# unslothai/unsloth

Measured on AMD Instinct MI355X. Metric: train tokens/sec, Llama-3-8B QLoRA (NF4) r=16 seq2048 bf16, higher is better.
Workload: dtype bf16; 1 GPU; Llama-3-8B QLoRA NF4 r=16 (q,k,v,o,gate,up,down) seq2048 bf16, fwd+bwd+AdamW; model=Llama-3-8B (synthetic weights), global_batch=4, seq_len=2048, parallelism=dp1, layers=32, lora_rank=16, gradient_checkpointing=unsloth, gc_schedule_chosen=all (every layer keeps everything), nf4_decoded_weight_mirrors=off (every NF4 weight is decoded at every use INSIDE the timed step), trainable_params=41943040, attention=csrc/attention.hip (causal GQA flash, fwd+bwd), optimizer=FlatAdamW fp32 on LoRA params

## Files before the change

### unsloth_amd/csrc/lora_side.hip

```cpp
#include "common.h"

typedef __attribute__((ext_vector_type(2))) __bf16 bf16x2_t;
typedef __attribute__((ext_vector_type(2))) _Float16 f16x2_t;

#define UAMD_TN_MAX_PROBLEMS 8

namespace {

constexpr int TN_COLS = 128;
constexpr int TN_R = 16;

struct TnArgs {
    int n_probs;
    int M;
    int S;
    int rows_per_wave;
    int total_slabs;
    int slab_start[UAMD_TN_MAX_PROBLEMS + 1];
    int64_t ws_off[UAMD_TN_MAX_PROBLEMS];
    float* ws;
    uamd_lora_tn_problem p[UAMD_TN_MAX_PROBLEMS];
};

typedef __attribute__((ext_vector_type(8))) __bf16 bf16x8_t;
typedef __attribute__((ext_vector_type(8))) _Float16 f16x8_t;
typedef __attribute__((ext_vector_type(4))) float f32x4_t;
typedef __attribute__((ext_vector_type(4))) short s16x4_t;
typedef __attribute__((address_space(3))) s16x4_t lds_s16x4;
typedef __attribute__((address_space(3))) unsigned char lds_u8;

template <typename T> struct Mfma16;
template <> struct Mfma16<bf16_t> {
    typedef bf16x8_t frag;
    static __device__ __forceinline__ f32x4_t run(frag a, frag b, f32x4_t c) {
        return __builtin_amdgcn_mfma_f32_16x16x32_bf16(a, b, c, 0, 0, 0);
    }
};
template <> struct Mfma16<f16_t> {
    typedef f16x8_t frag;
    static __device__ __forceinline__ f32x4_t run(frag a, frag b, f32x4_t c) {
        return __builtin_amdgcn_mfma_f32_16x16x32_f16(a, b, c, 0, 0, 0);
    }
};

constexpr int TN_ZT = 32 * 256;
constexpr int TN_PT = 32 * 64;
constexpr int TN_STAGE = TN_ZT + TN_PT;
#ifndef UAMD_TN_STAGES
#define UAMD_TN_STAGES 2
#endif
#ifndef UAMD_TN_RPW_MAX
#define UAMD_TN_RPW_MAX 512
#endif
#ifndef UAMD_TN_MIN_WAVES
#define UAMD_TN_MIN_WAVES 4096
#endif
constexpr int TN_NST = UAMD_TN_STAGES;
static_assert(TN_NST >= 2 && TN_NST <= 4, "ring of 2..4 stages (4 x 4 x 10 KiB = the 160 KiB of a CU)");
constexpr int TN_WAVE_LDS = TN_NST * TN_STAGE;

__device__ __forceinline__ void tn_dma(const void* gptr, unsigned lds_dst) {
    unsigned keep;
    asm volatile(
        "s_mov_b32 %0, m0\n\t"
        "s_mov_b32 m0, %2\n\t"
        "s_nop 0\n\t"
        "global_load_lds_dwordx4 %1, off\n\t"
        "s_mov_b32 m0, %0"
        : "=&s"(keep)
        : "v"(gptr), "s"(lds_dst)
        : "memory");
}

template <typename T>
__global__ void __launch_bounds__(256) lora_tn_kernel(TnArgs a) {
    extern __shared__ __attribute__((aligned(16))) unsigned char smem[];
    typedef typename Mfma16<T>::frag frag_t;
    const int tid = threadIdx.x, lane = tid & 63;
    const int wave = __builtin_amdgcn_readfirstlane(tid >> 6);
    const int64_t unit = (int64_t)blockIdx.x * 4 + wave;
    if (unit >= (int64_t)a.total_slabs * a.S) return;
    const int slab_lin = (int)(unit % a.total_slabs);
    const int sblk = (int)(unit / a.total_slabs);
    int pi = 0;
#pragma unroll
    for (int i = 1; i < UAMD_TN_MAX_PROBLEMS; ++i)
        if (i < a.n_probs && slab_lin >= a.slab_start[i]) pi = i;
    const uamd_lora_tn_problem& pr = a.p[pi];
    const int slab = slab_lin - a.slab_start[pi];
    const int n_slabs = a.slab_start[pi + 1] - a.slab_start[pi];
    const int M = a.M, N = pr.N, R = pr.R;
    const T* Z = (const T*)pr.Z;
    const float* P = pr.P;
    unsigned char* my = smem + wave * TN_WAVE_LDS;
    const unsigned my_lds = (unsigned)(uintptr_t)(lds_u8*)my;

    const int zr4 = lane >> 4;
    int zcol[8];
#pragma unroll
    for (int i = 0; i < 8; ++i) {
        const int row = 4 * i + zr4;
        const int f = (row & 3) | (((row >> 3) & 1) << 2);
        const int u16 = ((((lane & 15) >> 1) ^ f) << 1) | (lane & 1);
        int col = slab * TN_COLS + u16 * 8;
        if (col + 8 > N) col = N - 8;
        zcol[i] = col;
    }
    const int prow = lane >> 2;
    const int pc = (lane & 3) * 4 + 4 <= ((R + 3) & ~3) ? (lane & 3) * 4 : 0;
    auto issue = [&](int m0, int stage) {
        const unsigned d = my_lds + stage * TN_STAGE;
#pragma unroll
        for (int i = 0; i < 8; ++i) {
            int row = m0 + 4 * i + zr4;
            row = row < M ? row : M - 1;
            tn_dma(Z + (int64_t)row * pr.ldz + zcol[i], d + i * 1024);
        }
#pragma unroll
        for (int i = 0; i < 2; ++i) {
            int row = m0 + 16 * i + prow;
            row = row < M ? row : M - 1;
            tn_dma(P + (int64_t)row * pr.ldp + pc, d + TN_ZT + i * 1024);
        }
    };

    const int l15 = lane & 15, g4 = lane >> 4;
    const int sg2 = l15 >> 2;
    const int f_rd = sg2 | ((g4 & 1) << 2);
    const int z_lane = (8 * g4 + sg2) * 256 + f_rd * 32 + (l15 & 3) * 8;
    const int p_lane = TN_ZT + (8 * g4) * 64 + l15 * 4;

    f32x4_t acc[8];
#pragma unroll
    for (int j = 0; j < 8; ++j) acc[j] = f32x4_t{0.f, 0.f, 0.f, 0.f};

    const int m_base = sblk * a.rows_per_wave;
    const int m_end = min(m_base + a.rows_per_wave, M);
    const int nch = (m_end - m_base + 31) / 32;
#pragma unroll
    for (int i = 0; i < TN_NST - 1; ++i)
        if (i < nch) issue(m_base + 32 * i, i);
    for (int ch = 0; ch < nch; ++ch) {
        const int m0 = m_base + ch * 32;
        const int stage = ch % TN_NST;
        if (ch + TN_NST - 1 < nch) {
            issue(m0 + 32 * (TN_NST - 1), (ch + TN_NST - 1) % TN_NST);
            if (TN_NST == 2) asm volatile("s_waitcnt vmcnt(10)" ::: "memory");
            else if (TN_NST == 3) asm volatile("s_waitcnt vmcnt(20)" ::: "memory");
            else asm volatile("s_waitcnt vmcnt(30)" ::: "memory");
        } else {
            const int younger = nch - 1 - ch;
            if (younger >= 2) asm volatile("s_waitcnt vmcnt(20)" ::: "memory");
            else if (younger == 1) asm volatile("s_waitcnt vmcnt(10)" ::: "memory");
            else asm volatile("s_waitcnt vmcnt(0)" ::: "memory");
        }
        const unsigned char* sz = my + stage * TN_STAGE;
        union { T e[8]; frag_t f; } pa;
#pragma unroll
        for (int e = 0; e < 8; ++e) {
            float x = *reinterpret_cast<const float*>(sz + p_lane + e * 64);
            if (m0 + 8 * g4 + e >= M || l15 >= R) x = 0.f;
            pa.e[e] = from_f32<T>(x);
        }
#pragma unroll
        for (int jt = 0; jt < 8; ++jt) {
            union { s16x4_t h[2]; frag_t f; } zb;
            const int a0 = z_lane ^ (jt * 32);
            zb.h[0] = __builtin_amdgcn_ds_read_tr16_b64_v4i16((lds_s16x4*)(sz + a0));
            zb.h[1] = __builtin_amdgcn_ds_read_tr16_b64_v4i16((lds_s16x4*)(sz + a0 + 4 * 256));
            acc[jt] = Mfma16<T>::run(pa.f, zb.f, acc[jt]);
        }
    }

    const int64_t npad = (int64_t)n_slabs * TN_COLS;
    float* part = a.ws + a.ws_off[pi] + (int64_t)sblk * TN_R * npad + slab * TN_COLS + l15;
#pragma unroll
    for (int jt = 0; jt < 8; ++jt)
#pragma unroll
        for (int r = 0; r < 4; ++r) part[(int64_t)(4 * g4 + r) * npad + jt * 16] = acc[jt][r];
}

__global__ void __launch_bounds__(256) lora_tn_reduce_kernel(TnArgs a) {
    const int pi = blockIdx.y;
    const uamd_lora_tn_problem& pr = a.p[pi];
    const int n_slabs = a.slab_start[pi + 1] - a.slab_start[pi];
    const int64_t npad = (int64_t)n_slabs * TN_COLS;
    const int64_t idx = (int64_t)blockIdx.x * 256 + threadIdx.x;
    const int N = pr.N, R = pr.R;
    if (idx >= (int64_t)R * N) return;
    const int r = (int)(idx / N), n = (int)(idx - (int64_t)r * N);
    const float* part = a.ws + a.ws_off[pi] + (int64_t)r * npad + n;
    float v = 0.f;
    const int64_t sstride = (int64_t)TN_R * npad;
    int s = 0;
    for (; s + 8 <= a.S; s += 8) {
        float t[8];
#pragma unroll
        for (int u = 0; u < 8; ++u) t[u] = part[(int64_t)(s + u) * sstride];
#pragma unroll
        for (int u = 0; u < 8; ++u) v += t[u];
    }
    for (; s < a.S; ++s) v += part[(int64_t)s * sstride];
    v *= pr.scale;
    float* o = (pr.out_nr & 1) ? pr.out + (int64_t)n * pr.ldo + r : pr.out + (int64_t)r * pr.ldo + n;
    *o = (pr.out_nr & 2) ? *o + v : v;
}

constexpr int XA_KS = 64;
constexpr int XA_XT = 32 * XA_KS * 2;
template <int NT> struct XaCfg {
    static constexpr int WT = NT * 16 * XA_KS * 2;
    static constexpr int STAGE = XA_XT + WT;
    static constexpr int WAVE = 2 * STAGE;
    static constexpr int RED = 4 * 32 * NT * 16 * 4;
    static constexpr int LDS = 4 * WAVE > RED ? 4 * WAVE : RED;
};

template <typename T, int NT>
__global__ void __launch_bounds__(256) lora_xa2_kernel(const T* __restrict__ X, int64_t ldx,
                                                       const T* __restrict__ W, int64_t ldw,
                                                       float* __restrict__ out, int64_t ld_out,
                                                       T* __restrict__ out_k, int64_t ld_k, int k_cols,
                                                       int M, int K, int R, int out_cols) {
    extern __shared__ __attribute__((aligned(16))) unsigned char smem[];
    typedef typename Mfma16<T>::frag frag_t;
    typedef XaCfg<NT> C;
    const int tid = threadIdx.x, lane = tid & 63;
    const int wave = __builtin_amdgcn_readfirstlane(tid >> 6);
    const int l15 = lane & 15, g4 = lane >> 4;
    const int m0 = blockIdx.x * 32;
    unsigned char* my = smem + wave * C::WAVE;
    const unsigned my_lds = (unsigned)(uintptr_t)(lds_u8*)my;

    const int nsteps_all = (K + XA_KS - 1) / XA_KS;
    const int s_beg = (nsteps_all * wave) / 4, s_end = (nsteps_all * (wave + 1)) / 4;

    const int drow = lane >> 3;
    int xoff[4], woff[2 * NT];
    int xslot[4];
#pragma unroll
    for (int i = 0; i < 4; ++i) {
        const int row = 8 * i + drow;
        xslot[i] = (lane & 7) ^ ((row >> 1) & 7);
        int gm = m0 + row;
        gm = gm < M ? gm : M - 1;
        xoff[i] = gm;
    }
    int wslot[2 * NT];
#pragma unroll
    for (int i = 0; i < 2 * NT; ++i) {
        const int row = 8 * i + drow;
        wslot[i] = (lane & 7) ^ ((row >> 1) & 7);
        woff[i] = row < R ? row : R - 1;
    }
    auto issue = [&](int step, int stage) {
        const unsigned d = my_lds + stage * C::STAGE;
        const int k0 = step * XA_KS;
#pragma unroll
        for (int i = 0; i < 4; ++i) {
            int k = k0 + xslot[i] * 8;
            k = k + 8 <= K ? k : K - 8;
            tn_dma(X + (int64_t)xoff[i] * ldx + k, d + i * 1024);
        }
#pragma unroll
        for (int i = 0; i < 2 * NT; ++i) {
            int k = k0 + wslot[i] * 8;
            k = k + 8 <= K ? k : K - 8;
            tn_dma(W + (int64_t)woff[i] * ldw + k, d + XA_XT + i * 1024);
        }
    };

    f32x4_t acc[2][NT];
#pragma unroll
    for (int i = 0; i < 2; ++i)
#pragma unroll
        for (int j = 0; j < NT; ++j) acc[i][j] = f32x4_t{0.f, 0.f, 0.f, 0.f};

    const int sw = (l15 >> 1) & 7;
    const int f_lane = l15 * 128;
    constexpr int NDMA = 4 + 2 * NT;
    const int nst = s_end - s_beg;
    const int rot = nst > 0 ? (int)(blockIdx.x % nst) : 0;
    auto step_of = [&](int i) { const int j = i + rot; return s_beg + (j >= nst ? j - nst : j); };
    if (nst > 0) issue(step_of(0), 0);
    for (int it = 0; it < nst; ++it) {
        const int st = step_of(it);
        const int stage = it & 1;
        if (it + 1 < nst) {
            issue(step_of(it + 1), stage ^ 1);
            if (NDMA == 6) asm volatile("s_waitcnt vmcnt(6)" ::: "memory");
            else if (NDMA == 8) asm volatile("s_waitcnt vmcnt(8)" ::: "memory");
            else if (NDMA == 10) asm volatile("s_waitcnt vmcnt(10)" ::: "memory");
            else asm volatile("s_waitcnt vmcnt(12)" ::: "memory");
        } else {
            asm volatile("s_waitcnt vmcnt(0)" ::: "memory");
        }
        const unsigned char* sx = my + stage * C::STAGE;
        const unsigned char* swt = sx + XA_XT;
        const bool tail = st * XA_KS + XA_KS > K;
#pragma unroll
        for (int ks = 0; ks < 2; ++ks) {
            const int slot = ((4 * ks + g4) ^ sw) * 16;
            union FU { uint4 r; frag_t f; };
            FU xa[2], wb[NT];
#pragma unroll
            for (int i = 0; i < 2; ++i) xa[i].r = *reinterpret_cast<const uint4*>(sx + i * 2048 + f_lane + slot);
#pragma unroll
            for (int j = 0; j < NT; ++j) wb[j].r = *reinterpret_cast<const uint4*>(swt + j * 2048 + f_lane + slot);
            if (tail) {
                if (st * XA_KS + ks * 32 + g4 * 8 + 8 > K) {
#pragma unroll
                    for (int i = 0; i < 2; ++i) xa[i].r = make_uint4(0, 0, 0, 0);
                }
            }
#pragma unroll
            for (int i = 0; i < 2; ++i)
#pragma unroll
                for (int j = 0; j < NT; ++j) acc[i][j] = Mfma16<T>::run(xa[i].f, wb[j].f, acc[i][j]);
        }
    }

    __syncthreads();
    float* red = reinterpret_cast<float*>(smem);
#pragma unroll
    for (int i = 0; i < 2; ++i)
#pragma unroll
        for (int j = 0; j < NT; ++j)
#pragma unroll
            for (int r = 0; r < 4; ++r)
                red[(wave * 32 + i * 16 + 4 * g4 + r) * (NT * 16) + j * 16 + l15] = acc[i][j][r];
    __syncthreads();
    if (out != nullptr) {
        for (int idx = tid; idx < 32 * out_cols; idx += 256) {
            const int mm = idx / out_cols, c = idx - mm * out_cols;
            if (m0 + mm < M) {
                float v = 0.f;
                if (c < R) {
                    const float* q = red + mm * (NT * 16) + c;
                    v = ((q[0] + q[32 * NT * 16]) + q[2 * 32 * NT * 16]) + q[3 * 32 * NT * 16];
                }
                out[(int64_t)(m0 + mm) * ld_out + c] = v;
            }
        }
    }
    if (out_k != nullptr) {
        const int vec_per_row = k_cols >> 3;
        for (int idx = tid; idx < 32 * vec_per_row; idx += 256) {
            const int mm = idx / vec_per_row, c0 = (idx - mm * vec_per_row) * 8;
            if (m0 + mm < M) {
                Vec16<T> v;
#pragma unroll
                for (int j = 0; j < 8; ++j) {
                    const int c = c0 + j;
                    float x = 0.f;
                    if (c < R) {
                        const float* q = red + mm * (NT * 16) + c;
                        x = ((q[0] + q[32 * NT * 16]) + q[2 * 32 * NT * 16]) + q[3 * 32 * NT * 16];
                    }
                    v.e[j] = from_f32<T>(x);
                }
                st16(out_k + (int64_t)(m0 + mm) * ld_k + c0, v);
            }
        }
    }
}

template <typename T, int NT>
int launch_xa2(const void* X, int64_t ldx, const void* W, int64_t ldw, float* out, int64_t ld_out, void* out_k,
               int64_t ld_k, int k_cols, int M, int K, int R, int out_cols, hipStream_t st) {
    return uamd_launch_lds<&lora_xa2_kernel<T, NT>>(dim3((unsigned)((M + 31) / 32)), dim3(256), XaCfg<NT>::LDS, st, (const T*)X, ldx,
                                                    (const T*)W, ldw, out, ld_out, (T*)out_k, ld_k, k_cols, M, K, R, out_cols);
}

template <typename T>
int xa2_dispatch(const void* X, int64_t ldx, const void* W, int64_t ldw, float* out, int64_t ld_out, void* out_k,
                 int64_t ld_k, int k_cols, int M, int K, int R, int out_cols, hipStream_t st) {
    const int nt = (R + 15) / 16;
    if (nt <= 1) return launch_xa2<T, 1>(X, ldx, W, ldw, out, ld_out, out_k, ld_k, k_cols, M, K, R, out_cols, st);
    if (nt <= 2) return launch_xa2<T, 2>(X, ldx, W, ldw, out, ld_out, out_k, ld_k, k_cols, M, K, R, out_cols, st);
    if (nt <= 3) return launch_xa2<T, 3>(X, ldx, W, ldw, out, ld_out, out_k, ld_k, k_cols, M, K, R, out_cols, st);
    if (nt <= 4) return launch_xa2<T, 4>(X, ldx, W, ldw, out, ld_out, out_k, ld_k, k_cols, M, K, R, out_cols, st);
    return UAMD_ERR_ARG;
}

}

extern "C" int uamd_lora_tn(const uamd_lora_tn_problem* probs, int n_probs, int M, float* workspace,
                            int64_t workspace_floats, int dtype, void* stream) {
    if (!probs || n_probs < 1 || n_probs > UAMD_TN_MAX_PROBLEMS || M < 0 || !workspace) return UAMD_ERR_ARG;
    if (M == 0) return UAMD_OK;
    TnArgs a;
    a.n_probs = n_probs; a.M = M; a.ws = workspace;
    {
        int64_t slabs_all = 0;
        for (int i = 0; i < n_probs; ++i) slabs_all += (probs[i].N + TN_COLS - 1) / TN_COLS;
        int rpw = UAMD_TN_RPW_MAX;
        while (rpw > 128 && slabs_all * ((M + rpw - 1) / rpw) < UAMD_TN_MIN_WAVES) rpw >>= 1;
        a.rows_per_wave = rpw;
        a.S = (M + rpw - 1) / rpw;
    }
    int slabs = 0;
    int64_t off = 0;
    int max_rn_blocks = 1;
    for (int i = 0; i < UAMD_TN_MAX_PROBLEMS; ++i) {
        a.slab_start[i] = slabs;
        if (i < n_probs) {
            const uamd_lora_tn_problem& p = probs[i];
            if (!p.P || !p.Z || !p.out || p.N <= 0 || p.R <= 0 || p.R > TN_R) return UAMD_ERR_ARG;
            if ((p.N & 7) || p.N < 8 || (p.ldz & 7) || (p.ldp & 3) || !aligned16(p.Z) || !aligned16(p.P)) return UAMD_ERR_ALIGN;
            a.p[i] = p;
            a.ws_off[i] = off;
            const int ns = (p.N + TN_COLS - 1) / TN_COLS;
            slabs += ns;
            off += (int64_t)a.S * TN_R * ns * TN_COLS;
            const int64_t rn = ((int64_t)p.R * p.N + 255) / 256;
            if (rn > max_rn_blocks) max_rn_blocks = (int)rn;
        } else {
            a.p[i] = probs[0];
            a.ws_off[i] = 0;
        }
    }
    a.slab_start[UAMD_TN_MAX_PROBLEMS] = slabs;
    for (int i = n_probs; i < UAMD_TN_MAX_PROBLEMS; ++i) a.slab_start[i + 1] = slabs;
    a.total_slabs = slabs;
    if (off > workspace_floats) return UAMD_ERR_ARG;
    const int64_t blocks = ((int64_t)slabs * a.S + 3) / 4;
    if (blocks > 0x7fffffffLL) return UAMD_ERR_ARG;
    hipStream_t st = (hipStream_t)stream;
    UAMD_DISPATCH_HALF(dtype,
        if (int rc = uamd_launch_lds<&lora_tn_kernel<T>>(dim3((unsigned)blocks), dim3(256), 4 * TN_WAVE_LDS, st, a)) return rc)
    hipLaunchKernelGGL(lora_tn_reduce_kernel, dim3((unsigned)max_rn_blocks, (unsigned)n_probs), dim3(256), 0, st, a);
    return uamd_launch_status();
}

extern "C" int uamd_lora_xa2k(const void* X, int64_t ldx, const void* W, int64_t ldw, float* out, int64_t ld_out,
                              void* out_k, int64_t ld_k, int k_cols, int M, int K, int R, int out_cols, int dtype,
                              void* stream) {
    if (M < 0 || K < 8 || R <= 0 || R > 64) return UAMD_ERR_ARG;
    if (!out && !out_k) return UAMD_ERR_ARG;
    if (out && (out_cols < R || out_cols > 256)) return UAMD_ERR_ARG;
    if (out_k && (k_cols < R || k_cols > 256)) return UAMD_ERR_ARG;
    if (M == 0) return UAMD_OK;
    if ((K & 7) || (ldx & 7) || (ldw & 7) || !aligned16(X) || !aligned16(W)) return UAMD_ERR_ALIGN;
    if (out_k && ((k_cols & 7) || (ld_k & 7) || !aligned16(out_k))) return UAMD_ERR_ALIGN;
    UAMD_DISPATCH_HALF(dtype, return xa2_dispatch<T>(X, ldx, W, ldw, out, ld_out, out_k, ld_k, k_cols, M, K, R, out_cols, (hipStream_t)stream))
    return UAMD_ERR_DTYPE;
}

extern "C" int uamd_lora_xa2(const void* X, int64_t ldx, const void* W, int64_t ldw, float* out, int64_t ld_out,
                             int M, int K, int R, int out_cols, int dtype, void* stream) {
    if (!out) return UAMD_ERR_ARG;
    return uamd_lora_xa2k(X, ldx, W, ldw, out, ld_out, nullptr, 0, 0, M, K, R, out_cols, dtype, stream);
}

namespace {
template <typename T>
__global__ void __launch_bounds__(256) lora_prepare_kernel(const uamd_lora_prep_desc* __restrict__ d, int n_mats,
                                                          const int* __restrict__ tile_prefix) {
    __shared__ float tile[32][33];
    int lo = 0, hi = n_mats - 1;
    const int bid = blockIdx.x;
    while (lo < hi) {
        const int mid = (lo + hi + 1) >> 1;
        if (tile_prefix[mid] <= bid) lo = mid; else hi = mid - 1;
    }
    const uamd_lora_prep_desc m = d[lo];
    const int t = bid - tile_prefix[lo];
    const int tiles_c = (m.cols + 31) / 32;
    const int r0 = (t / tiles_c) * 32, c0 = (t % tiles_c) * 32;
    const int tx = threadIdx.x & 31, ty = threadIdx.x >> 5;
    const float* src = (const float*)m.src;
    T* rm = (T*)m.dst_rowmajor;
    T* tr = (T*)m.dst_transposed;
    T* pad = (T*)m.dst_pad;
    const bool pad_t = m.pad_transposed != 0;
#pragma unroll
    for (int i = 0; i < 4; ++i) {
        const int r = r0 + ty + 8 * i, c = c0 + tx;
        float v = 0.f;
        if (r < m.rows && c < m.cols) {
            v = src[(int64_t)r * m.cols + c];
            if (rm) rm[(int64_t)r * m.cols + c] = from_f32<T>(v);
            if (pad && !pad_t) pad[(int64_t)r * m.pad_ld + c] = from_f32<T>(m.pad_scale * v);
        }
        tile[ty + 8 * i][tx] = v;
    }
    __syncthreads();
    if (tr || (pad && pad_t)) {
#pragma unroll
        for (int i = 0; i < 4; ++i) {
            const int c = c0 + ty + 8 * i, r = r0 + tx;
            if (r < m.rows && c < m.cols) {
                const float v = tile[tx][ty + 8 * i];
                if (tr) tr[(int64_t)c * m.rows + r] = from_f32<T>(v);
                if (pad && pad_t) pad[(int64_t)c * m.pad_ld + r] = from_f32<T>(m.pad_scale * v);
            }
        }
    }
}
}

extern "C" int uamd_lora_prepare(const uamd_lora_prep_desc* descs_dev, const int* tile_prefix_dev, int n_mats,
                                 int total_tiles, int dtype, void* stream) {
    if (!descs_dev || !tile_prefix_dev || n_mats <= 0 || total_tiles < 0) return UAMD_ERR_ARG;
    if (total_tiles == 0) return UAMD_OK;
    hipStream_t st = (hipStream_t)stream;
    UAMD_DISPATCH_HALF(dtype, hipLaunchKernelGGL((lora_prepare_kernel<T>), dim3((unsigned)total_tiles), dim3(256), 0, st, descs_dev, n_mats,
                                                 tile_prefix_dev))
    return uamd_launch_status();
}
```

Baseline: 37580 tokens/s.

## Group LoRA TN problems sharing the same Z operand into one walk

When three LoRA weight-gradient problems share the same Z matrix (e.g. q/k/v using the same input activations), the TN kernel now streams Z through LDS once and runs three MFMA accumulators against it. The extra P operands are loaded straight from global memory into registers. This cuts redundant Z reads and the number of waves, at the cost of more registers (3x8 accumulators plus P values) and fewer units to spread across the GPU. A tuning bit can switch the grouping off.

```diff
diff --git a/unsloth_amd/csrc/lora_side.hip b/unsloth_amd/csrc/lora_side.hip
--- a/unsloth_amd/csrc/lora_side.hip
+++ b/unsloth_amd/csrc/lora_side.hip
@@ -10,13 +10,17 @@
 constexpr int TN_COLS = 128;
 constexpr int TN_R = 16;
 
+constexpr int TN_GROUP = 3;
+
 struct TnArgs {
     int n_probs;
+    int n_walks;
     int M;
     int S;
     int rows_per_wave;
     int total_slabs;
-    int slab_start[UAMD_TN_MAX_PROBLEMS + 1];
+    int walk_start[UAMD_TN_MAX_PROBLEMS + 1];
+    int walk_mem[UAMD_TN_MAX_PROBLEMS];
     int64_t ws_off[UAMD_TN_MAX_PROBLEMS];
     float* ws;
     uamd_lora_tn_problem p[UAMD_TN_MAX_PROBLEMS];
@@ -72,27 +76,24 @@
         : "memory");
 }
 
-template <typename T>
-__global__ void __launch_bounds__(256) lora_tn_kernel(TnArgs a) {
-    extern __shared__ __attribute__((aligned(16))) unsigned char smem[];
+__device__ __forceinline__ float tn_ldg(const float* p) {
+    float v;
+    asm volatile("global_load_dword %0, %1, off" : "=v"(v) : "v"(p) : "memory");
+    return v;
+}
+__device__ __forceinline__ void tn_landed(float (&x)[8]) {
+    asm volatile("" : "+v"(x[0]), "+v"(x[1]), "+v"(x[2]), "+v"(x[3]), "+v"(x[4]), "+v"(x[5]), "+v"(x[6]), "+v"(x[7]));
+}
+
+template <typename T, int NM>
+__device__ __forceinline__ void tn_unit(const TnArgs& a, const int (&mem)[TN_GROUP], int slab, int n_slabs, int sblk,
+                                        unsigned char* my, int lane) {
     typedef typename Mfma16<T>::frag frag_t;
-    const int tid = threadIdx.x, lane = tid & 63;
-    const int wave = __builtin_amdgcn_readfirstlane(tid >> 6);
-    const int64_t unit = (int64_t)blockIdx.x * 4 + wave;
-    if (unit >= (int64_t)a.total_slabs * a.S) return;
-    const int slab_lin = (int)(unit % a.total_slabs);
-    const int sblk = (int)(unit / a.total_slabs);
-    int pi = 0;
-#pragma unroll
-    for (int i = 1; i < UAMD_TN_MAX_PROBLEMS; ++i)
-        if (i < a.n_probs && slab_lin >= a.slab_start[i]) pi = i;
-    const uamd_lora_tn_problem& pr = a.p[pi];
-    const int slab = slab_lin - a.slab_start[pi];
-    const int n_slabs = a.slab_start[pi + 1] - a.slab_start[pi];
-    const int M = a.M, N = pr.N, R = pr.R;
+    const uamd_lora_tn_problem& pr = a.p[mem[0]];
+    const int M = a.M, N = pr.N;
     const T* Z = (const T*)pr.Z;
     const float* P = pr.P;
-    unsigned char* my = smem + wave * TN_WAVE_LDS;
+    const int R0 = pr.R;
     const unsigned my_lds = (unsigned)(uintptr_t)(lds_u8*)my;
 
     const int zr4 = lane >> 4;
@@ -107,7 +108,7 @@
         zcol[i] = col;
     }
     const int prow = lane >> 2;
-    const int pc = (lane & 3) * 4 + 4 <= ((R + 3) & ~3) ? (lane & 3) * 4 : 0;
+    const int pc = (lane & 3) * 4 + 4 <= ((R0 + 3) & ~3) ? (lane & 3) * 4 : 0;
     auto issue = [&](int m0, int stage) {
         const unsigned d = my_lds + stage * TN_STAGE;
 #pragma unroll
@@ -130,9 +131,23 @@
     const int z_lane = (8 * g4 + sg2) * 256 + f_rd * 32 + (l15 & 3) * 8;
     const int p_lane = TN_ZT + (8 * g4) * 64 + l15 * 4;
 
-    f32x4_t acc[8];
-#pragma unroll
-    for (int j = 0; j < 8; ++j) acc[j] = f32x4_t{0.f, 0.f, 0.f, 0.f};
+    const float* pk[NM];
+    int64_t ldpk[NM];
+    int Rk[NM];
+    Rk[0] = R0;
+#pragma unroll
+    for (int k = 1; k < NM; ++k) {
+        const uamd_lora_tn_problem& q = a.p[mem[k]];
+        Rk[k] = q.R;
+        ldpk[k] = q.ldp;
+        pk[k] = q.P + (l15 < q.R ? l15 : q.R - 1);
+    }
+
+    f32x4_t acc[NM][8];
+#pragma unroll
+    for (int k = 0; k < NM; ++k)
+#pragma unroll
+        for (int j = 0; j < 8; ++j) acc[k][j] = f32x4_t{0.f, 0.f, 0.f, 0.f};
 
     const int m_base = sblk * a.rows_per_wave;
     const int m_end = min(m_base + a.rows_per_wave, M);
@@ -143,6 +158,15 @@
     for (int ch = 0; ch < nch; ++ch) {
         const int m0 = m_base + ch * 32;
         const int stage = ch % TN_NST;
+        float px[NM][8];
+#pragma unroll
+        for (int k = 1; k < NM; ++k)
+#pragma unroll
+            for (int e = 0; e < 8; ++e) {
+                int row = m0 + 8 * g4 + e;
+                row = row < M ? row : M - 1;
+                px[k][e] = tn_ldg(pk[k] + (int64_t)row * ldpk[k]);
+            }
         if (ch + TN_NST - 1 < nch) {
             issue(m0 + 32 * (TN_NST - 1), (ch + TN_NST - 1) % TN_NST);
             if (TN_NST == 2) asm volatile("s_waitcnt vmcnt(10)" ::: "memory");
@@ -154,39 +178,72 @@
             else if (younger == 1) asm volatile("s_waitcnt vmcnt(10)" ::: "memory");
             else asm volatile("s_waitcnt vmcnt(0)" ::: "memory");
         }
+#pragma unroll
+        for (int k = 1; k < NM; ++k) tn_landed(px[k]);
         const unsigned char* sz = my + stage * TN_STAGE;
-        union { T e[8]; frag_t f; } pa;
-#pragma unroll
-        for (int e = 0; e < 8; ++e) {
-            float x = *reinterpret_cast<const float*>(sz + p_lane + e * 64);
-            if (m0 + 8 * g4 + e >= M || l15 >= R) x = 0.f;
-            pa.e[e] = from_f32<T>(x);
-        }
+        union { T e[8]; frag_t f; } pa[NM];
+#pragma unroll
+        for (int e = 0; e < 8; ++e) px[0][e] = *reinterpret_cast<const float*>(sz + p_lane + e * 64);
+        if constexpr (NM > 1) tn_landed(px[0]);
+#pragma unroll
+        for (int k = 0; k < NM; ++k)
+#pragma unroll
+            for (int e = 0; e < 8; ++e) {
+                float x = px[k][e];
+                if (m0 + 8 * g4 + e >= M || l15 >= Rk[k]) x = 0.f;
+                pa[k].e[e] = from_f32<T>(x);
+            }
 #pragma unroll
         for (int jt = 0; jt < 8; ++jt) {
             union { s16x4_t h[2]; frag_t f; } zb;
             const int a0 = z_lane ^ (jt * 32);
             zb.h[0] = __builtin_amdgcn_ds_read_tr16_b64_v4i16((lds_s16x4*)(sz + a0));
             zb.h[1] = __builtin_amdgcn_ds_read_tr16_b64_v4i16((lds_s16x4*)(sz + a0 + 4 * 256));
-            acc[jt] = Mfma16<T>::run(pa.f, zb.f, acc[jt]);
+#pragma unroll
+            for (int k = 0; k < NM; ++k) acc[k][jt] = Mfma16<T>::run(pa[k].f, zb.f, acc[k][jt]);
         }
     }
 
     const int64_t npad = (int64_t)n_slabs * TN_COLS;
-    float* part = a.ws + a.ws_off[pi] + (int64_t)sblk * TN_R * npad + slab * TN_COLS + l15;
-#pragma unroll
-    for (int jt = 0; jt < 8; ++jt)
-#pragma unroll
-        for (int r = 0; r < 4; ++r) part[(int64_t)(4 * g4 + r) * npad + jt * 16] = acc[jt][r];
+#pragma unroll
+    for (int k = 0; k < NM; ++k) {
+        float* part = a.ws + a.ws_off[mem[k]] + (int64_t)sblk * TN_R * npad + slab * TN_COLS + l15;
+#pragma unroll
+        for (int jt = 0; jt < 8; ++jt)
+#pragma unroll
+            for (int r = 0; r < 4; ++r) part[(int64_t)(4 * g4 + r) * npad + jt * 16] = acc[k][jt][r];
+    }
+}
+
+template <typename T>
+__global__ void __launch_bounds__(256) lora_tn_kernel(TnArgs a) {
+    extern __shared__ __attribute__((aligned(16))) unsigned char smem[];
+    const int tid = threadIdx.x, lane = tid & 63;
+    const int wave = __builtin_amdgcn_readfirstlane(tid >> 6);
+    const int64_t unit = (int64_t)blockIdx.x * 4 + wave;
+    if (unit >= (int64_t)a.total_slabs * a.S) return;
+    const int slab_lin = (int)(unit % a.total_slabs);
+    const int sblk = (int)(unit / a.total_slabs);
+    int w = 0;
+#pragma unroll
+    for (int i = 1; i < UAMD_TN_MAX_PROBLEMS; ++i)
+        if (i < a.n_walks && slab_lin >= a.walk_start[i]) w = i;
+    const int slab = slab_lin - a.walk_start[w];
+    const int n_slabs = a.walk_start[w + 1] - a.walk_start[w];
+    unsigned char* my = smem + wave * TN_WAVE_LDS;
+    const int wm = a.walk_mem[w];
+    const int mem[TN_GROUP] = {wm & 15, (wm >> 4) & 15, (wm >> 8) & 15};
+    const int nm = wm >> 12;
+    if (nm == TN_GROUP) tn_unit<T, TN_GROUP>(a, mem, slab, n_slabs, sblk, my, lane);
+    else tn_unit<T, 1>(a, mem, slab, n_slabs, sblk, my, lane);
 }
 
 __global__ void __launch_bounds__(256) lora_tn_reduce_kernel(TnArgs a) {
     const int pi = blockIdx.y;
     const uamd_lora_tn_problem& pr = a.p[pi];
-    const int n_slabs = a.slab_start[pi + 1] - a.slab_start[pi];
-    const int64_t npad = (int64_t)n_slabs * TN_COLS;
+    const int N = pr.N, R = pr.R;
+    const int64_t npad = (int64_t)((N + TN_COLS - 1) / TN_COLS) * TN_COLS;
     const int64_t idx = (int64_t)blockIdx.x * 256 + threadIdx.x;
-    const int N = pr.N, R = pr.R;
     if (idx >= (int64_t)R * N) return;
     const int r = (int)(idx / N), n = (int)(idx - (int64_t)r * N);
     const float* part = a.ws + a.ws_off[pi] + (int64_t)r * npad + n;
@@ -399,20 +456,16 @@
         a.rows_per_wave = rpw;
         a.S = (M + rpw - 1) / rpw;
     }
-    int slabs = 0;
     int64_t off = 0;
     int max_rn_blocks = 1;
     for (int i = 0; i < UAMD_TN_MAX_PROBLEMS; ++i) {
-        a.slab_start[i] = slabs;
         if (i < n_probs) {
             const uamd_lora_tn_problem& p = probs[i];
             if (!p.P || !p.Z || !p.out || p.N <= 0 || p.R <= 0 || p.R > TN_R) return UAMD_ERR_ARG;
             if ((p.N & 7) || p.N < 8 || (p.ldz & 7) || (p.ldp & 3) || !aligned16(p.Z) || !aligned16(p.P)) return UAMD_ERR_ALIGN;
             a.p[i] = p;
             a.ws_off[i] = off;
-            const int ns = (p.N + TN_COLS - 1) / TN_COLS;
-            slabs += ns;
-            off += (int64_t)a.S * TN_R * ns * TN_COLS;
+            off += (int64_t)a.S * TN_R * ((p.N + TN_COLS - 1) / TN_COLS) * TN_COLS;
             const int64_t rn = ((int64_t)p.R * p.N + 255) / 256;
             if (rn > max_rn_blocks) max_rn_blocks = (int)rn;
         } else {
@@ -420,10 +473,29 @@
             a.ws_off[i] = 0;
         }
     }
-    a.slab_start[UAMD_TN_MAX_PROBLEMS] = slabs;
-    for (int i = n_probs; i < UAMD_TN_MAX_PROBLEMS; ++i) a.slab_start[i + 1] = slabs;
+    if (off > workspace_floats) return UAMD_ERR_ARG;
+    const bool grouping = (uamd_tuning_get(UAMD_TUNE_STREAM_NT) & 4) == 0;
+    bool taken[UAMD_TN_MAX_PROBLEMS] = {false};
+    int slabs = 0, n_walks = 0;
+    for (int i = 0; i < n_probs; ++i) {
+        if (taken[i]) continue;
+        int found[TN_GROUP] = {i}, nm = 1;
+        for (int j = i + 1; grouping && j < n_probs && nm < TN_GROUP; ++j)
+            if (!taken[j] && probs[j].Z == probs[i].Z && probs[j].ldz == probs[i].ldz && probs[j].N == probs[i].N) found[nm++] = j;
+        int mem = i;
+        if (nm == TN_GROUP) {
+            for (int k = 1; k < TN_GROUP; ++k) { taken[found[k]] = true; mem |= found[k] << (4 * k); }
+        } else {
+            nm = 1;
+        }
+        a.walk_start[n_walks] = slabs;
+        a.walk_mem[n_walks++] = mem | (nm << 12);
+        slabs += (probs[i].N + TN_COLS - 1) / TN_COLS;
+    }
+    for (int w = n_walks; w < UAMD_TN_MAX_PROBLEMS; ++w) { a.walk_start[w] = slabs; a.walk_mem[w] = 1 << 12; }
+    a.walk_start[UAMD_TN_MAX_PROBLEMS] = slabs;
+    a.n_walks = n_walks;
     a.total_slabs = slabs;
-    if (off > workspace_floats) return UAMD_ERR_ARG;
     const int64_t blocks = ((int64_t)slabs * a.S + 3) / 4;
     if (blocks > 0x7fffffffLL) return UAMD_ERR_ARG;
     hipStream_t st = (hipStream_t)stream;
```

After: 37550 tokens/s. About the same (-0.1%).
